# unirestore/UniRestore

Measured on AMD Instinct MI355X. Metric: restored 512x512 images/sec @ 20 denoise steps (whole job), higher is better.
Workload: dtype bf16; 1 GPU; PIR 512x512 batch=8/GPU, 20 DDIM steps, bf16, hipGraph replay (BASELINE.json configs[1]; configs[2] shape for N=8); global_batch=8, per_gpu_batch=8, image=512, denoise_steps=20, parallelism=image-parallel dp1, weights=seeded random init (no checkpoints reachable)

## Files before the change

### unirestore_amd/csrc/igemm.hip

```cpp
#include "igemm_impl.h"

namespace urk {
#define UR_DECLARE(name)                                                                                             \
  ConvLaunch name##_bf16(void* k, size_t ws_bytes);                                                                 \
  ConvLaunch name##_f16(void* k, size_t ws_bytes);                                                                  \
  static ConvLaunch name(ConvK& k, size_t ws_bytes) { return (k.f16 ? name##_f16 : name##_bf16)(&k, ws_bytes); }
UR_CONV_LAUNCHERS(UR_DECLARE)
#undef UR_DECLARE
}

namespace {

ConvLaunch dispatch_conv(ConvK& k, bool pair, size_t ws_bytes) {
  k.fold = 0;
  if (k.w4 && k.ups && k.KH == 3 && k.stride == 1 && k.pad_t == 1 && k.pad_l == 1 && k.kcm && k.staged_ok_ && !pair && k.nbatch == 1 &&
      k.C2 == 0 && k.Cin % 64 == 0 && k.W % 32 == 0 && k.H % 8 == 0 && k.OH == 2 * k.H && k.OW == 2 * k.W && !k.yt && !k.gn_ab && !k.row_stats &&
      !k.ln_stats) {
    k.fold = 1;
    const long long tm = 4ll * k.N * (k.H / 8) * (k.W / 32);
    auto fill = [](long long t) { return (double)t / (double)(((t + 255) / 256) * 256); };
    const bool ok128 = k.Cout % 128 == 0, ok160 = k.Cout % 160 == 0;
    if (ok160 && (!ok128 || fill(tm * (k.Cout / 160)) >= fill(tm * (k.Cout / 128)))) return urk::halo_8x32_160(k, ws_bytes);
    return urk::halo_8x32_128(k, ws_bytes);
  }
  if (k.KH == 3 && k.stride == 1 && k.pad_t == 1 && k.pad_l == 1 && k.kcm && k.staged_ok_ && !pair && k.nbatch == 1 &&
      k.OW % 32 == 0 && k.OH % 8 == 0 && k.OH == (k.ups ? 2 * k.H : k.H) && k.OW == (k.ups ? 2 * k.W : k.W) && !k.yt) {
    const bool ok128 = k.Cout % 128 == 0, ok160 = k.Cout % 160 == 0;
    const long long tm8 = (long long)k.N * (k.OH / 8) * (k.OW / 32);
    auto eff = [](long long t) { return t <= 128 ? (double)(t * (256 / t)) / 256.0 : (double)t / (double)(((t + 255) / 256) * 256); };
    const bool use160 = ok160 && (!ok128 || eff(tm8 * (k.Cout / 160)) >= eff(tm8 * (k.Cout / 128)));
    const long long tiles8 = tm8 * (use160 ? k.Cout / 160 : k.Cout / 128);
    if ((ok128 || ok160) && tiles8 >= 64) {
      if (use160) return urk::halo_8x32_160(k, ws_bytes);
      return urk::halo_8x32_128(k, ws_bytes);
    }
  }
  if (k.KH == 3 && k.stride == 1 && k.pad_t == 1 && k.pad_l == 1 && k.kcm && !pair && k.nbatch == 1 && !k.ups && k.C2 == 0 &&
      k.Cout <= 32 && k.OW % 32 == 0 && k.OH % 8 == 0 && k.OH == k.H && k.OW == k.W && !k.yt && !k.gn_part && !k.gn_ab && !k.row_stats && !k.ln_stats &&
      !k.bias_img && (long long)k.N * (k.OH / 8) * (k.OW / 32) >= 128)
    return urk::halo_thin_32(k, ws_bytes);
  const bool himg_ups = k.ups && k.OH == 16 && k.OW == 16 && k.H == 8 && k.W == 8;
  if (k.KH == 3 && k.stride == 1 && k.pad_t == 1 && k.pad_l == 1 && k.kcm && k.staged_ok_ && !pair && k.nbatch == 1 &&
      ((!k.ups && k.OH == k.H && k.OW == k.W) || himg_ups) && !k.yt && k.Cout % 128 == 0 && k.nk >= 36) {
    if (k.wf && k.OH == 8 && k.OW == 8 && k.N <= 16 && k.Cin % 256 == 0 && k.nk >= 72 && k.y && k.ws && !k.gn_ab && !k.row_stats && !k.ln_stats &&
        (long long)(k.nk / 36) * k.M * k.Cout * 4 <= (long long)ws_bytes)
      return urk::wstream_8x8(k, ws_bytes);
    if (k.OH == 16 && k.OW == 16) return urk::himg_16x16(k, ws_bytes);
    if (k.OH == 8 && k.OW == 8 && k.N % 4 == 0) {
      return urk::himg_8x8x4(k, ws_bytes);
    }
// ... 220 lines not shown
```

### unirestore_amd/csrc/igemm_impl.h

```cpp
#pragma once
#include <cstdio>
#include <cstdlib>
#include <map>
#include <string>

#include "common.h"

static __device__ uint4 g_zero_page[8];
typedef uint32_t ig_u32x4 __attribute__((ext_vector_type(4)));

struct ConvLaunch {
  int (*launch)(void* k, hipStream_t s);
  int prologue_ok;
  int id;
};

namespace {

struct ConvK {
  const uint16_t* x; const uint16_t* x2; const uint16_t* w; const float* bias; const uint16_t* res;
  void* y; uint16_t* yt; float* ws; float* gn_part; const float* gn_ab;
  float* row_stats; const float* ln_stats; const float* ln_colsum; float ln_eps; int ln_dim, ln_parts;
  int N, H, W, C1, ldx, C2, ldx2, Cin, Cout, ldw, ldy, ldr, KH, KW, stride, pad_t, pad_l, OH, OW, OHW;
  int ups, act, out_f32, n_split, t_rows, t_ld;
// ... 1862 lines not shown
    static ur::DeviceOnce attr_once;
    if (auto once_guard = attr_once.first()) {
      hipFuncSetAttribute(reinterpret_cast<const void*>(&igemm_halo_kernel<TH, BN, WM, WN, UR_TU_F16 != 0, false>), hipFuncAttributeMaxDynamicSharedMemorySize, lds);
      hipFuncSetAttribute(reinterpret_cast<const void*>(&igemm_halo_kernel<TH, BN, WM, WN, UR_TU_F16 != 0, GN_OK>), hipFuncAttributeMaxDynamicSharedMemorySize, lds);
      hipFuncSetAttribute(reinterpret_cast<const void*>(&igemm_halo_ws_kernel<TH, BN, WM, WN, UR_TU_F16 != 0, false>), hipFuncAttributeMaxDynamicSharedMemorySize, lds);
      hipFuncSetAttribute(reinterpret_cast<const void*>(&igemm_halo_ws_kernel<TH, BN, WM, WN, UR_TU_F16 != 0, GN_OK>), hipFuncAttributeMaxDynamicSharedMemorySize, lds);
      hipFuncSetAttribute(reinterpret_cast<const void*>(&igemm_halo_kernel<TH, BN, WM, WN, UR_TU_F16 != 0, false, 4>), hipFuncAttributeMaxDynamicSharedMemorySize, lds);
      hipFuncSetAttribute(reinterpret_cast<const void*>(&igemm_halo_ws_kernel<TH, BN, WM, WN, UR_TU_F16 != 0, false, 4>), hipFuncAttributeMaxDynamicSharedMemorySize, lds);
    }
    static const bool no_ws = getenv("UR_HALO_NOWS") != nullptr;
    if (k.fold) {
      const dim3 grid(k.tiles_m * k.tiles_n, 4);
      if (no_ws) UR_F16_SWITCH(k, hipLaunchKernelGGL((igemm_halo_kernel<TH, BN, WM, WN, F16, false, 4>), grid, dim3(NW * 64), lds, s, k));
      else UR_F16_SWITCH(k, hipLaunchKernelGGL((igemm_halo_ws_kernel<TH, BN, WM, WN, F16, false, 4>), grid, dim3((NW + 2) * 64), lds, s, k));
      return ur::check_launch("ur_conv2d_nhwc");
    }
    if (no_ws) {
      if (GN_OK && k.gn_ab) UR_F16_SWITCH(k, hipLaunchKernelGGL((igemm_halo_kernel<TH, BN, WM, WN, F16, GN_OK>), dim3(k.tiles_m * k.tiles_n, k.splitk), dim3(NW * 64), lds, s, k));
      else UR_F16_SWITCH(k, hipLaunchKernelGGL((igemm_halo_kernel<TH, BN, WM, WN, F16, false>), dim3(k.tiles_m * k.tiles_n, k.splitk), dim3(NW * 64), lds, s, k));
    } else {
      static const bool ld1 = getenv("UR_HALO_LD1") != nullptr;
      const dim3 blk((NW + (ld1 ? 1 : 2)) * 64);
      if (GN_OK && k.gn_ab) UR_F16_SWITCH(k, hipLaunchKernelGGL((igemm_halo_ws_kernel<TH, BN, WM, WN, F16, GN_OK>), dim3(k.tiles_m * k.tiles_n, k.splitk), blk, lds, s, k));
      else UR_F16_SWITCH(k, hipLaunchKernelGGL((igemm_halo_ws_kernel<TH, BN, WM, WN, F16, false>), dim3(k.tiles_m * k.tiles_n, k.splitk), blk, lds, s, k));
    }
    if (k.splitk > 1) {
      k.patch_tw = 0;
      launch_splitk_reduce(k, s);
    }
    return ur::check_launch("ur_conv2d_nhwc");
  }
};

template <int TH, int TW, int NIMG, int BN, int WM, int WN, bool F16, bool GNP>
__global__ __launch_bounds__(WM* WN * 64) void igemm_halo_img_kernel(const ConvK p) {
  constexpr int NW = WM * WN, BM = TH * TW * NIMG, PW = TW + 2, HP = (TH + 2) * PW, HPIX = HP * NIMG;
  constexpr int HSLOTS = (HPIX + 8 * NW - 1) / (8 * NW);
  constexpr int HPIECES = HSLOTS * NW, HBYTES = HPIECES * 1024;
  constexpr int WBYTES = BN * 128, WPIECES = BN / 8, WPW = (WPIECES + NW - 1) / NW;
  constexpr int WTM = BM / WM, WTN = BN / WN, FM = WTM / 32, FN = WTN / 32, NT = NW * 64;
  static_assert(BM == 256 && NW == 8 && WTM % 32 == 0 && WTN % 32 == 0 && HSLOTS <= 8, "tile shape");
  extern __shared__ __attribute__((aligned(16))) unsigned char smem[];
  unsigned char* const hbuf = smem;
  unsigned char* const wring = smem + 2 * HBYTES;
  unsigned char* const abuf = wring + 3 * WBYTES;
  constexpr bool GN_OK = NIMG == 1 && HSLOTS <= 7;
  constexpr bool gnp = GN_OK && GNP;

  const int tid = threadIdx.x, lane = tid & 63, wid = tid >> 6;
  const int wm = wid % WM, wn = wid / WM;
  int sz = blockIdx.y, tn, tmi;
  if (p.wmajor) {
    const int L = blockIdx.x, xcd = L & 7, j = L >> 3;
    const int g = (j / p.tiles_m) * 8 + xcd;
    if (g >= p.tiles_n * p.splitk) return;
    tn = g % p.tiles_n; sz = g / p.tiles_n; tmi = j % p.tiles_m;
  } else {
    int id = blockIdx.x;
    const int nt = p.tiles_m * p.tiles_n, q = nt >> 3, r = nt & 7, xcd = id & 7, idx = id >> 3;
    id = (xcd < r ? xcd * (q + 1) : r * (q + 1) + (xcd - r) * q) + idx;
    tn = id % p.tiles_n; tmi = id / p.tiles_n;
  }
  const int n0 = tn * BN, img0 = tmi * NIMG, m0 = tmi * BM;

  typedef __attribute__((address_space(1))) const void* gptr_t;
  typedef __attribute__((address_space(3))) void* lptr_t;
  const uint16_t* __restrict__ X1 = p.x;
  const uint16_t* __restrict__ X2 = p.x2;
  const uint16_t* __restrict__ Wt = p.w;
  const uint16_t* zero = reinterpret_cast<const uint16_t*>(g_zero_page);
  const int lr = lane >> 3, ps = lane & 7;

  int hpix[HSLOTS], hchk[HSLOTS];
#pragma unroll
  for (int t = 0; t < HSLOTS; ++t) {
    const int hr = (t * NW + wid) * 8 + lr;
    const int im = hr / HP, rin = hr - im * HP, hy = rin / PW, hx = rin - hy * PW;
    const int iy = hy - 1, ix = hx - 1;
    const bool v = hr < HPIX && img0 + im < p.N && (unsigned)iy < (unsigned)TH && (unsigned)ix < (unsigned)TW;
    const int sy = p.ups ? iy >> 1 : iy, sx = p.ups ? ix >> 1 : ix;
    hpix[t] = v ? ((img0 + im) * p.H + sy) * p.W + sx : -1;
    hchk[t] = ps ^ (((rin >> 1) - hy) & 7);
  }
  const int wchunk = ps ^ ((((wid & 1) << 2) + (lr >> 1)) & 7);
  int woff[WPW];
#pragma unroll
  for (int i = 0; i < WPW; ++i) {
    const int qq = (wid + NW * i < WPIECES) ? wid + NW * i : wid;
    const int row = n0 + qq * 8 + lr;
    woff[i] = row < p.Cout ? row * p.ldw : -1;
  }
  const int nchunk_all = p.nk / 9, cps = p.nk_per_split / 9;
  const int c_begin = sz * cps, c_end = min(nchunk_all, c_begin + cps);
  const int nchunk = c_end - c_begin, nk = nchunk * 9, kt0 = c_begin * 9;

  const int wid_s = __builtin_amdgcn_readfirstlane(wid);
  const ig_u32x4 rs_w = ig_make_rsrc(Wt, (unsigned long long)p.Cout * p.ldw * 2);
  const ig_u32x4 rs_x1 = ig_make_rsrc(X1, (unsigned long long)p.N * p.H * p.W * p.ldx * 2);
  const ig_u32x4 rs_x2 = ig_make_rsrc(X2 ? X2 : X1, (unsigned long long)p.N * p.H * p.W * (X2 ? p.ldx2 : p.ldx) * 2);
  const unsigned wring_lds = (unsigned)(uintptr_t)(lptr_t)wring, hbuf_lds = (unsigned)(uintptr_t)(lptr_t)hbuf;
  unsigned wvo[WPW];
#pragma unroll
  for (int i = 0; i < WPW; ++i) wvo[i] = woff[i] >= 0 ? (unsigned)woff[i] * 2u + wchunk * 16u : IG_OOB;
  auto issue_w = [&](int kt, int ring) {
#pragma unroll
    for (int i = 0; i < WPW; ++i) {
      const int qq = (wid_s + NW * i < WPIECES) ? wid_s + NW * i : wid_s;
      ig_lds_dma16(wring_lds + ring * WBYTES + qq * 1024, wvo[i], rs_w, (unsigned)(kt0 + kt) * 128u);
    }
  };
  auto issue_h = [&](int c, int t) {
    const int cb = (c_begin + c) * 64;
    const bool second = cb >= p.C1;
    const unsigned ld2 = (unsigned)(second ? p.ldx2 : p.ldx) * 2u;
    const unsigned vo = hpix[t] >= 0 ? (unsigned)hpix[t] * ld2 + hchk[t] * 16u : IG_OOB;
    const unsigned m0v = hbuf_lds + (c & 1) * HBYTES + (t * NW + wid_s) * 1024;
    if (second) ig_lds_dma16(m0v, vo, rs_x2, (unsigned)(cb - p.C1) * 2u);
    else ig_lds_dma16(m0v, vo, rs_x1, (unsigned)cb * 2u);
  };
  auto issue_ab = [&](int c) {
    const float* t = p.gn_ab + ((long long)img0 * 2 + (lane >> 4 & 1)) * p.Cin + (c_begin + c) * 64 + (lane & 15) * 4;
    const void* g = lane < 32 ? (const void*)t : (const void*)zero;
    __builtin_amdgcn_global_load_lds((gptr_t)g, (lptr_t)(abuf + (c & 1) * 1024), 16, 0, 0);
  };
  auto gn_slot = [&](int c, int t) {
    if (hpix[t] >= 0)
      gn_piece_inplace<F16>(hbuf + (c & 1) * HBYTES + (t * NW + wid) * 1024 + lane * 16, gn_load_ab(abuf + (c & 1) * 1024, hchk[t]), p.gn_silu != 0);
  };

  f32x16 acc[FN][FM];
// ... 4 lines not shown
#pragma unroll
      for (int e = 0; e < 16; ++e) acc[a][b][e] = 0.f;
  const int frow = lane & 31, fhalf = lane >> 5;
  int hrow0[FM], hin0[FM], hy0[FM];
#pragma unroll
  for (int b = 0; b < FM; ++b) {
    const int pix = wm * WTM + b * 32 + frow;
    const int im = pix / (TH * TW), r = pix - im * (TH * TW), y = r / TW, x = r - y * TW;
    hin0[b] = y * PW + x;
    hrow0[b] = im * HP + hin0[b];
    hy0[b] = y;
  }
  const unsigned hb_lds = (unsigned)(uintptr_t)(lptr_t)hbuf;
  const unsigned aw_lds = (unsigned)(uintptr_t)(lptr_t)wring + (wn * WTN + frow) * 128 + ((fhalf ^ ((frow >> 1) & 7)) << 4);
  static_assert(((WTN >> 1) & 7) == 0, "the wave's weight rows must keep the swizzle phase of fragment row 0");

  if (gnp) issue_ab(0);
#pragma unroll
  for (int t = 0; t < HSLOTS; ++t) issue_h(0, t);
  issue_w(0, 0);
  if (nk > 1) {
    issue_w(1, 1);
    asm volatile("s_waitcnt vmcnt(%0)" ::"n"(WPW) : "memory");
  } else {
    asm volatile("s_waitcnt vmcnt(0)" ::: "memory");
  }
  if (gnp) {
#pragma unroll
    for (int t = 0; t < HSLOTS; ++t) gn_slot(0, t);
    asm volatile("s_waitcnt lgkmcnt(0)" ::: "memory");
  }
  __builtin_amdgcn_s_barrier();

  for (int c = 0; c < nchunk; ++c) {
    const unsigned char* hb = hbuf + (c & 1) * HBYTES;
    const bool next_chunk = c + 1 < nchunk;
#pragma unroll
    for (int tap = 0; tap < 9; ++tap) {
      const int kt = c * 9 + tap;
      const bool more_w = kt + 2 < nk;
      const bool more_h = tap < HSLOTS && next_chunk;
      if (more_w) issue_w(kt + 2, (tap + 2) % 3);
      if (tap < HSLOTS) { if (next_chunk) issue_h(c + 1, tap < HSLOTS ? tap : 0); }
      const bool ab_now = gnp && tap == 0 && next_chunk;
      if (ab_now) issue_ab(c + 1);
      if (gnp && tap >= 2 && tap - 2 < HSLOTS && next_chunk) gn_slot(c + 1, (tap >= 2 && tap - 2 < HSLOTS) ? tap - 2 : 0);
      if constexpr (ktile_asm_ok<FM, FN>()) {
        const int dy = tap / 3, dx = tap % 3;
        unsigned ab[FM];
#pragma unroll
        for (int b = 0; b < FM; ++b) {
          const int hsw = (((hin0[b] + dy * PW + dx) >> 1) - (hy0[b] + dy)) & 7;
          ab[b] = hb_lds + (c & 1) * HBYTES + (hrow0[b] + dy * PW + dx) * 128 + ((fhalf ^ hsw) << 4);
        }
        ktile_mma<FM, FN, F16>(acc, ab, aw_lds + (tap % 3) * WBYTES);
      } else {
        const int dy = tap / 3, dx = tap % 3;
        const unsigned char* wsm = wring + (tap % 3) * WBYTES;
        int hro[FM], hsw[FM];
#pragma unroll
        for (int b = 0; b < FM; ++b) {
          hro[b] = (hrow0[b] + dy * PW + dx) * 128;
          hsw[b] = (((hin0[b] + dy * PW + dx) >> 1) - (hy0[b] + dy)) & 7;
        }
#pragma unroll
        for (int ks = 0; ks < 4; ++ks) {
          const int slot = ks * 2 + fhalf;
          typename Frag<F16>::type bfr[FM], afr[FN];
#pragma unroll
          for (int b = 0; b < FM; ++b) bfr[b] = *reinterpret_cast<const typename Frag<F16>::type*>(hb + hro[b] + ((slot ^ hsw[b]) << 4));
#pragma unroll
          for (int a = 0; a < FN; ++a) {
            const int row = wn * WTN + a * 32 + frow;
            afr[a] = *reinterpret_cast<const typename Frag<F16>::type*>(wsm + row * 128 + ((slot ^ ((row >> 1) & 7)) << 4));
          }
#pragma unroll
          for (int a = 0; a < FN; ++a)
#pragma unroll
            for (int b = 0; b < FM; ++b)
              acc[a][b] = mfma16t(afr[a], bfr[b], acc[a][b]);
        }
      }
      if (ab_now) {
        if (more_w) asm volatile("s_waitcnt vmcnt(%0)" ::"n"(WPW + 2) : "memory");
        else asm volatile("s_waitcnt vmcnt(2)" ::: "memory");
      } else if (more_w && more_h) asm volatile("s_waitcnt vmcnt(%0)" ::"n"(WPW + 1) : "memory");
      else if (more_w) asm volatile("s_waitcnt vmcnt(%0)" ::"n"(WPW) : "memory");
      else if (more_h) asm volatile("s_waitcnt vmcnt(1)" ::: "memory");
      else asm volatile("s_waitcnt vmcnt(0)" ::: "memory");
      asm volatile("s_waitcnt lgkmcnt(0)" ::: "memory");
      __builtin_amdgcn_s_barrier();
    }
  }
  asm volatile("s_nop 15\n\ts_nop 7" ::: "memory");
  igemm_epilogue<FM, FN, WTM, WTN, BM, BN, NT, F16, false>(p, acc, m0, n0, wm, wn, lane, 0, sz, smem);
}

template <int TH, int TW, int NIMG, int BN, int WM, int WN, bool F16>
__global__ __launch_bounds__((WM * WN + 2) * 64) void igemm_halo_img_ws_kernel(const ConvK p) {
  constexpr int NW = WM * WN, BM = TH * TW * NIMG, PW = TW + 2, HP = (TH + 2) * PW, HPIX = HP * NIMG;
  constexpr int HSLOTS = (HPIX + 8 * NW - 1) / (8 * NW);
  constexpr int HPIECES = HSLOTS * NW, HBYTES = HPIECES * 1024;
  constexpr int WBYTES = BN * 128, WPIECES = BN / 8;
  constexpr int WTM = BM / WM, WTN = BN / WN, FM = WTM / 32, FN = WTN / 32, NT = NW * 64;
  static_assert(BM == 256 && NW == 8 && WTM % 32 == 0 && WTN % 32 == 0 && HSLOTS <= 8 && ktile_asm_ok<FM, FN>() && WPIECES % NW == 0, "tile shape");
  extern __shared__ __attribute__((aligned(16))) unsigned char smem[];
  unsigned char* const hbuf = smem;
  unsigned char* const wring = smem + 2 * HBYTES;
  typedef __attribute__((address_space(3))) void* lptr_t;

  const int tid = threadIdx.x, lane = tid & 63, wid = tid >> 6;
  const int wid_s = __builtin_amdgcn_readfirstlane(wid);
  int sz = blockIdx.y, tn, tmi;
  if (p.wmajor) {
    const int L = blockIdx.x, xcd = L & 7, j = L >> 3;
    const int g = (j / p.tiles_m) * 8 + xcd;
    if (g >= p.tiles_n * p.splitk) return;
    tn = g % p.tiles_n; sz = g / p.tiles_n; tmi = j % p.tiles_m;
  } else {
    int id = blockIdx.x;
    const int nt = p.tiles_m * p.tiles_n, q = nt >> 3, r = nt & 7, xcd = id & 7, idx = id >> 3;
    id = (xcd < r ? xcd * (q + 1) : r * (q + 1) + (xcd - r) * q) + idx;
    tn = id % p.tiles_n; tmi = id / p.tiles_n;
  }
  const int n0 = tn * BN, img0 = tmi * NIMG, m0 = tmi * BM;
  const int lr = lane >> 3, ps = lane & 7;
  const int nchunk_all = p.nk / 9, cps = p.nk_per_split / 9;
  const int c_begin = sz * cps, c_end = min(nchunk_all, c_begin + cps);
  const int nchunk = c_end - c_begin, nk = nchunk * 9, kt0 = c_begin * 9;
  const ig_u32x4 rs_w = ig_make_rsrc(p.w, (unsigned long long)p.Cout * p.ldw * 2);
  const ig_u32x4 rs_x1 = ig_make_rsrc(p.x, (unsigned long long)p.N * p.H * p.W * p.ldx * 2);
  const ig_u32x4 rs_x2 = ig_make_rsrc(p.x2 ? p.x2 : p.x, (unsigned long long)p.N * p.H * p.W * (p.x2 ? p.ldx2 : p.ldx) * 2);
  const unsigned wring_lds = (unsigned)(uintptr_t)(lptr_t)wring, hbuf_lds = (unsigned)(uintptr_t)(lptr_t)hbuf;

  auto piece_of = [&](int q, int& pix, int& chk) {
    const int hr = q * 8 + lr;
    const int im = hr / HP, rin = hr - im * HP, hy = rin / PW, hx = rin - hy * PW;
    const int iy = hy - 1, ix = hx - 1;
    const bool v = hr < HPIX && img0 + im < p.N && (unsigned)iy < (unsigned)TH && (unsigned)ix < (unsigned)TW;
    const int sy = p.ups ? iy >> 1 : iy, sx = p.ups ? ix >> 1 : ix;
    pix = v ? ((img0 + im) * p.H + sy) * p.W + sx : -1;
    chk = ps ^ (((rin >> 1) - hy) & 7);
  };
  auto dma_piece = [&](int c, int q, int pix, int chk) {
    const int cb = (c_begin + c) * 64;
    const bool second = cb >= p.C1;
    const unsigned ld2 = (unsigned)(second ? p.ldx2 : p.ldx) * 2u;
    const unsigned vo = pix >= 0 ? (unsigned)pix * ld2 + chk * 16u : IG_OOB;
    const unsigned m0v = hbuf_lds + (c & 1) * HBYTES + q * 1024;
    if (second) ig_lds_dma16(m0v, vo, rs_x2, (unsigned)(cb - p.C1) * 2u);
    else ig_lds_dma16(m0v, vo, rs_x1, (unsigned)cb * 2u);
  };
  auto wvo_of = [&](int q) -> unsigned {
    const int row = n0 + q * 8 + lr;
    const int wchunk = ps ^ ((((q & 1) << 2) + (lr >> 1)) & 7);
    return row < p.Cout ? (unsigned)row * (unsigned)p.ldw * 2u + wchunk * 16u : IG_OOB;
  };

  if (wid_s == NW) {
    unsigned wvo[WPIECES];
#pragma unroll
    for (int q = 0; q < WPIECES; ++q) wvo[q] = wvo_of(q);
    auto dma_w = [&](int kt, int ring) {
      const unsigned so = (unsigned)(kt0 + kt) * 128u;
#pragma unroll
      for (int q = 0; q < WPIECES; ++q) ig_lds_dma16(wring_lds + ring * WBYTES + q * 1024, wvo[q], rs_w, so);
    };
    if (nk > 1) dma_w(1, 1);
    asm volatile("s_waitcnt vmcnt(0)" ::: "memory");
    __builtin_amdgcn_s_barrier();
    for (int kt = 0; kt < nk; ++kt) {
      if (kt + 2 < nk) {
        dma_w(kt + 2, (kt + 2) % 3);
        asm volatile("s_waitcnt vmcnt(%0)" ::"n"(WPIECES) : "memory");
      } else {
        asm volatile("s_waitcnt vmcnt(0)" ::: "memory");
      }
      __builtin_amdgcn_s_barrier();
    }
    return;
  }
  if (wid_s == NW + 1) {
    int hpx[HPIECES];
#pragma unroll
    for (int q = 0; q < HPIECES; ++q) { int pix, chk; piece_of(q, pix, chk); hpx[q] = pix >= 0 ? pix * 8 + chk : -1; }
    __builtin_amdgcn_s_barrier();
    constexpr int PPT = (HPIECES + 7) / 8;
    for (int c = 0; c < nchunk; ++c) {
      const bool next_chunk = c + 1 < nchunk;
#pragma unroll
      for (int tap = 0; tap < 9; ++tap) {
        if (next_chunk && tap < 8) {
#pragma unroll
          for (int j = 0; j < PPT; ++j) {
            const int q = tap * PPT + j;
            if (q < HPIECES) dma_piece(c + 1, q, hpx[q < HPIECES ? q : 0] >= 0 ? hpx[q < HPIECES ? q : 0] >> 3 : -1, hpx[q < HPIECES ? q : 0] & 7);
          }
        }
        if (tap == 8 || !next_chunk) asm volatile("s_waitcnt vmcnt(0)" ::: "memory");
        else asm volatile("s_waitcnt vmcnt(%0)" ::"n"(PPT) : "memory");
        __builtin_amdgcn_s_barrier();
      }
    }
    return;
  }

  const int wm = wid % WM, wn = wid / WM;
  {
#pragma unroll
    for (int t = 0; t < HSLOTS; ++t) { int pix, chk; piece_of(t * NW + wid_s, pix, chk); dma_piece(0, t * NW + wid_s, pix, chk); }
#pragma unroll
    for (int i = 0; i < WPIECES / NW; ++i) ig_lds_dma16(wring_lds + (wid_s + NW * i) * 1024, wvo_of(wid_s + NW * i), rs_w, (unsigned)kt0 * 128u);
  }
  f32x16 acc[FN][FM];
#pragma unroll
  for (int a = 0; a < FN; ++a)
#pragma unroll
    for (int b = 0; b < FM; ++b)
#pragma unroll
      for (int e = 0; e < 16; ++e) acc[a][b][e] = 0.f;
  const int frow = lane & 31, fhalf = lane >> 5;
  int hrow0[FM], hin0[FM], hy0[FM];
#pragma unroll
  for (int b = 0; b < FM; ++b) {
    const int pix = wm * WTM + b * 32 + frow;
    const int im = pix / (TH * TW), r = pix - im * (TH * TW), y = r / TW, x = r - y * TW;
    hin0[b] = y * PW + x;
    hrow0[b] = im * HP + hin0[b];
    hy0[b] = y;
  }
  const unsigned aw_lds = wring_lds + (wn * WTN + frow) * 128 + ((fhalf ^ ((frow >> 1) & 7)) << 4);
  static_assert(((WTN >> 1) & 7) == 0, "the wave's weight rows must keep the swizzle phase of fragment row 0");
  asm volatile("s_waitcnt vmcnt(0)" ::: "memory");
  __builtin_amdgcn_s_barrier();
  for (int c = 0; c < nchunk; ++c) {
#pragma unroll
    for (int tap = 0; tap < 9; ++tap) {
      const int dy = tap / 3, dx = tap % 3;
      unsigned ab[FM];
#pragma unroll
      for (int b = 0; b < FM; ++b) {
        const int hsw = (((hin0[b] + dy * PW + dx) >> 1) - (hy0[b] + dy)) & 7;
        ab[b] = hbuf_lds + (c & 1) * HBYTES + (hrow0[b] + dy * PW + dx) * 128 + ((fhalf ^ hsw) << 4);
      }
      ktile_mma<FM, FN, F16>(acc, ab, aw_lds + (tap % 3) * WBYTES);
      asm volatile("s_waitcnt lgkmcnt(0)" ::: "memory");
      __builtin_amdgcn_s_barrier();
    }
  }
  asm volatile("s_nop 15\n\ts_nop 7" ::: "memory");
  igemm_epilogue<FM, FN, WTM, WTN, BM, BN, NT, F16, false>(p, acc, m0, n0, wm, wn, lane, 0, sz, smem);
}

template <int TH, int TW, int NIMG, int BN, int WM, int WN>
struct HaloImg {
  static constexpr int NW = WM * WN, BM = TH * TW * NIMG, HPIX = (TH + 2) * (TW + 2) * NIMG, HSLOTS = (HPIX + 8 * NW - 1) / (8 * NW);
  static constexpr int HBYTES = HSLOTS * NW * 1024;
  static constexpr bool GN_OK = NIMG == 1 && HSLOTS <= 7;
  static constexpr int lds_loop = 2 * HBYTES + 3 * BN * 128 + (GN_OK ? 2048 : 0), lds_epi = epi_lds_bytes<BM, BN, NW * 64>();
  static constexpr int lds = lds_loop > lds_epi ? lds_loop : lds_epi;
  static_assert(lds <= 160 * 1024, "LDS budget");
  static int plan(ConvK& k, size_t ws_bytes) {
    k.tiles_m = (k.N + NIMG - 1) / NIMG;
    k.tiles_n = (k.Cout + BN - 1) / BN;
    const int nchunk = k.nk / 9;
    const long long tiles = (long long)k.tiles_m * k.tiles_n;
    plan_splitk(k, ws_bytes, tiles < 200 && k.ws && k.y ? std::min<long long>(std::max<long long>(256 / tiles, 1), std::max(1, nchunk / 2)) : 1, 9);
    set_gn_plan(k, (k.OHW % BM) == 0, k.OHW / BM);
    return GN_OK;
  }
  static int launch(ConvK& k, hipStream_t s) {
    static ur::DeviceOnce attr_once;
    if (auto once_guard = attr_once.first()) {
      hipFuncSetAttribute(reinterpret_cast<const void*>(&igemm_halo_img_kernel<TH, TW, NIMG, BN, WM, WN, UR_TU_F16 != 0, false>), hipFuncAttributeMaxDynamicSharedMemorySize, lds);
      hipFuncSetAttribute(reinterpret_cast<const void*>(&igemm_halo_img_kernel<TH, TW, NIMG, BN, WM, WN, UR_TU_F16 != 0, GN_OK>), hipFuncAttributeMaxDynamicSharedMemorySize, lds);
    }
    static const bool no_wmajor = getenv("UR_HIMG_NOWMAJOR") != nullptr;
    const int slices = k.tiles_n * k.splitk, per_xcd = ((slices + 7) / 8) * k.tiles_m;
    k.wmajor = !no_wmajor && (long long)k.Cout * k.Ktot > (long long)k.N * k.H * k.W * k.Cin && per_xcd <= 32 && slices >= 8;
    const dim3 grid = k.wmajor ? dim3(8 * per_xcd, 1) : dim3(k.tiles_m * k.tiles_n, k.splitk);
    static const bool himg_ws = getenv("UR_HIMG_NOWS") == nullptr;
    if (himg_ws && !k.gn_ab) {
      static ur::DeviceOnce ws_once;
      if (auto g2 = ws_once.first())
        hipFuncSetAttribute(reinterpret_cast<const void*>(&igemm_halo_img_ws_kernel<TH, TW, NIMG, BN, WM, WN, UR_TU_F16 != 0>), hipFuncAttributeMaxDynamicSharedMemorySize, lds);
      UR_F16_SWITCH(k, hipLaunchKernelGGL((igemm_halo_img_ws_kernel<TH, TW, NIMG, BN, WM, WN, F16>), grid, dim3((NW + 2) * 64), lds, s, k));
    } else if (GN_OK && k.gn_ab) UR_F16_SWITCH(k, hipLaunchKernelGGL((igemm_halo_img_kernel<TH, TW, NIMG, BN, WM, WN, F16, GN_OK>), grid, dim3(NW * 64), lds, s, k));
    else UR_F16_SWITCH(k, hipLaunchKernelGGL((igemm_halo_img_kernel<TH, TW, NIMG, BN, WM, WN, F16, false>), grid, dim3(NW * 64), lds, s, k));
    if (k.splitk > 1) launch_splitk_reduce(k, s);
    return ur::check_launch("ur_conv2d_nhwc");
  }
};

}
```

### unirestore_amd/ops.py

```python
from dataclasses import dataclass
from typing import Optional

import torch

from . import capi
from .capi import (UR_ACT_GATE, UR_ACT_GEGLU, UR_ACT_GELU, UR_ACT_NONE, UR_ACT_RELU, UR_ACT_SILU, UR_ACT_TANH, UR_DT_BF16,
                   UR_DT_F16, ConvDesc, ConvPlan, check, lib)

BF16 = torch.bfloat16
F16 = torch.float16
_ws = {}

_DTYPES = {"bf16": BF16, "bfloat16": BF16, BF16: BF16, "fp16": F16, "float16": F16, "f16": F16, "16": F16, F16: F16}
_act = BF16


def set_dtype(dt) -> torch.dtype:
    global _act
    if dt not in _DTYPES:
        raise ValueError(f"unsupported compute dtype {dt!r}: choose 'bf16' or 'fp16'")
    _act = _DTYPES[dt]
    return _act


def act_dtype() -> torch.dtype:
    return _act


def _dt(t: Optional[torch.Tensor] = None) -> int:
    d = _act if t is None else t.dtype
    if d == BF16:
        return UR_DT_BF16
# ... 58 lines not shown
        if self.w_frag is None:
            nt, nc = self.cout // 128, self.cin // 64
            w = self.w.view(nt, 4, 32, nc, 9, 4, 2, 8)
            self.w_frag = w.permute(0, 3, 4, 5, 1, 6, 2, 7).contiguous()
        return self.w_frag

    w_up4: Optional[torch.Tensor] = None

    def up4(self, weight: torch.Tensor) -> torch.Tensor:
        if self.w_up4 is None:
            w = weight.detach().to(self.w.device, torch.float32).permute(0, 2, 3, 1)
            if w.shape[0] != self.cout or w.shape[3] != self.cin:
                w = torch.nn.functional.pad(w, (0, self.cin - w.shape[3], 0, 0, 0, 0, 0, self.cout - w.shape[0]))
            self.w_up4 = up4_pack(up4_fold(w), self.w.dtype)
        return self.w_up4


def up4_fold(w: torch.Tensor) -> torch.Tensor:
    sel = w.new_tensor([[[1, 0, 0], [0, 1, 1]], [[1, 1, 0], [0, 0, 1]]])
    return torch.einsum("pay,qbx,oyxc->pqoabc", sel, sel, w)


def up4_pack(w4: torch.Tensor, dtype) -> torch.Tensor:
    _, _, cout, _, _, cin = w4.shape
    assert cin % 64 == 0
    return w4.to(dtype).reshape(4, cout, 4, cin // 64, 64).permute(0, 1, 3, 2, 4).reshape(4, cout, 4 * cin).contiguous()


def up4_unpack(packed: torch.Tensor, cin: int) -> torch.Tensor:
    cout = packed.shape[1]
    return packed.reshape(2, 2, cout, cin // 64, 2, 2, 64).permute(0, 1, 2, 4, 5, 3, 6).reshape(2, 2, cout, 2, 2, cin)


def wants_up4(pc: "PackedConv", n, h, w_, c1, c2, stride, upsample, groups, pad=(1, 1)) -> bool:
    return (pc.k == 3 and pc.kcm and groups == 1 and stride == 1 and bool(upsample) and tuple(pad) == (1, 1) and not pc.pair
            and c2 == 0 and c1 % 64 == 0 and w_ % 32 == 0 and h % 8 == 0)


def wants_frag(pc: "PackedConv", n, h, w_, c1, c2, stride, upsample, groups) -> bool:
    return (pc.k == 3 and pc.kcm and groups == 1 and stride == 1 and not upsample and h == 8 and w_ == 8 and n <= 16 and not pc.pair
            and pc.cout % 128 == 0 and (c1 + c2) % 256 == 0 and (c1 + c2) >= 512 and (c2 == 0 or c1 % 64 == 0))


def pack_conv(weight: torch.Tensor, bias: Optional[torch.Tensor], dev, *, pair=False, groups=1, cin_pad=None, c1=None, group_halo=False) -> PackedConv:
    w = weight.detach().to(dev, torch.float32)
    if w.dim() == 2:
        w = w[:, :, None, None]
    cout, cin_g, kh, kw = w.shape
    assert kh == kw and kh in (1, 3)
    cin_p = cin_pad or round_up(cin_g, 8)
    cout_p = round_up(cout, 8)
    if groups > 1:
        assert cin_g % 8 == 0 and (cout // groups) % 4 == 0
    if cin_p == cin_g and cout_p == cout:
        wp = w.permute(0, 2, 3, 1).contiguous()
    else:
        wp = torch.zeros(cout_p, kh, kw, cin_p, dtype=torch.float32, device=dev)
        wp[:cout, :, :, :cin_g] = w.permute(0, 2, 3, 1)
    b = None
    if bias is not None:
        b = torch.zeros(cout_p, dtype=torch.float32, device=dev)
        b[:cout] = bias.detach().to(dev, torch.float32)
    cout_out = cout_p
    if pair:
        half = cout // 2
        if cout % 2 or half % 32:
            raise NotImplementedError(f"UR_E_UNSUPPORTED: pair activations (GEGLU / SimpleGate) need (Cout/2) % 32 == 0, got {half}")
        idx = torch.arange(cout, device=dev).view(2, half // 32, 32).permute(1, 0, 2).reshape(-1)
        wp = wp[idx]
# ... 1024 lines not shown
```

Before: 30.43 images/s.

## Extend folded 4-tap upsample conv to 16x16 inputs via whole-image halo kernel

Adds a 4-tap phase-decomposed (nearest-upsample folded) variant of the whole-image halo implicit-GEMM kernels. For 16x16 inputs with Cin>=256 it is selected when enough workgroups exist. Each of the four output phases runs a 2x2 conv on the low-resolution input instead of a 3x3 conv on the upsampled image, which cuts MACs by about 9/4 and shrinks halo loads. The trade-offs are extra weight packing, new vmcnt wait cases and a rotating weight-ring index, plus a heuristic threshold that decides when the fold is worth it.

```diff
diff --git a/unirestore_amd/csrc/igemm.hip b/unirestore_amd/csrc/igemm.hip
--- a/unirestore_amd/csrc/igemm.hip
+++ b/unirestore_amd/csrc/igemm.hip
@@ -13,9 +13,16 @@
 
 ConvLaunch dispatch_conv(ConvK& k, bool pair, size_t ws_bytes) {
   k.fold = 0;
-  if (k.w4 && k.ups && k.KH == 3 && k.stride == 1 && k.pad_t == 1 && k.pad_l == 1 && k.kcm && k.staged_ok_ && !pair && k.nbatch == 1 &&
-      k.C2 == 0 && k.Cin % 64 == 0 && k.W % 32 == 0 && k.H % 8 == 0 && k.OH == 2 * k.H && k.OW == 2 * k.W && !k.yt && !k.gn_ab && !k.row_stats &&
-      !k.ln_stats) {
+  const bool fold_ok = k.w4 && k.ups && k.KH == 3 && k.stride == 1 && k.pad_t == 1 && k.pad_l == 1 && k.kcm && k.staged_ok_ && !pair && k.nbatch == 1 &&
+                       k.C2 == 0 && k.Cin % 64 == 0 && k.OH == 2 * k.H && k.OW == 2 * k.W && !k.yt && !k.gn_ab && !k.row_stats && !k.ln_stats;
+  if (fold_ok && k.H == 16 && k.W == 16 && k.Cin >= 256 && himg_up4_bn(k)) {
+    static const int min_wgs = getenv("UR_HIMG_FOLD_MIN") ? atoi(getenv("UR_HIMG_FOLD_MIN")) : 80;
+    if (4ll * k.N * (k.Cout / himg_up4_bn(k)) >= min_wgs || k.Cin <= 320) {
+      k.fold = 1;
+      return urk::himg_16x16(k, ws_bytes);
+    }
+  }
+  if (fold_ok && k.W % 32 == 0 && k.H % 8 == 0) {
     k.fold = 1;
     const long long tm = 4ll * k.N * (k.H / 8) * (k.W / 32);
     auto fill = [](long long t) { return (double)t / (double)(((t + 255) / 256) * 256); };
diff --git a/unirestore_amd/csrc/igemm_impl.h b/unirestore_amd/csrc/igemm_impl.h
--- a/unirestore_amd/csrc/igemm_impl.h
+++ b/unirestore_amd/csrc/igemm_impl.h
@@ -1918,8 +1918,10 @@
   }
 };
 
-template <int TH, int TW, int NIMG, int BN, int WM, int WN, bool F16, bool GNP>
+template <int TH, int TW, int NIMG, int BN, int WM, int WN, bool F16, bool GNP, int NTAP = 9>
 __global__ __launch_bounds__(WM* WN * 64) void igemm_halo_img_kernel(const ConvK p) {
+  constexpr bool UP4 = NTAP == 4;
+  static_assert((NTAP == 9 || NTAP == 4) && !(UP4 && (GNP || NIMG != 1)), "tap count");
   constexpr int NW = WM * WN, BM = TH * TW * NIMG, PW = TW + 2, HP = (TH + 2) * PW, HPIX = HP * NIMG;
   constexpr int HSLOTS = (HPIX + 8 * NW - 1) / (8 * NW);
   constexpr int HPIECES = HSLOTS * NW, HBYTES = HPIECES * 1024;
@@ -1932,6 +1934,8 @@
   unsigned char* const abuf = wring + 3 * WBYTES;
   constexpr bool GN_OK = NIMG == 1 && HSLOTS <= 7;
   constexpr bool gnp = GN_OK && GNP;
+  constexpr int HPT = UP4 ? (HSLOTS + NTAP - 2) / (NTAP - 1) : 1;
+  static_assert(HPT <= 2, "vmcnt cases of the tap wait");
 
   const int tid = threadIdx.x, lane = tid & 63, wid = tid >> 6;
   const int wm = wid % WM, wn = wid / WM;
@@ -1939,7 +1943,7 @@
   if (p.wmajor) {
     const int L = blockIdx.x, xcd = L & 7, j = L >> 3;
     const int g = (j / p.tiles_m) * 8 + xcd;
-    if (g >= p.tiles_n * p.splitk) return;
+    if (g >= p.tiles_n * (UP4 ? 4 : p.splitk)) return;
     tn = g % p.tiles_n; sz = g / p.tiles_n; tmi = j % p.tiles_m;
   } else {
     int id = blockIdx.x;
@@ -1947,13 +1951,16 @@
     id = (xcd < r ? xcd * (q + 1) : r * (q + 1) + (xcd - r) * q) + idx;
     tn = id % p.tiles_n; tmi = id / p.tiles_n;
   }
-  const int n0 = tn * BN, img0 = tmi * NIMG, m0 = tmi * BM;
+  const int phase = UP4 ? sz : 0, py = phase >> 1, px = phase & 1;
+  if constexpr (UP4) sz = 0;
+  const int n0 = tn * BN, img0 = tmi * NIMG, m0 = UP4 ? up4_m0(p, img0, 0, 0, TH, TW, py) : tmi * BM;
+  const int ldw = UP4 ? 4 * p.Cin : p.ldw;
 
   typedef __attribute__((address_space(1))) const void* gptr_t;
   typedef __attribute__((address_space(3))) void* lptr_t;
   const uint16_t* __restrict__ X1 = p.x;
   const uint16_t* __restrict__ X2 = p.x2;
-  const uint16_t* __restrict__ Wt = p.w;
+  const uint16_t* __restrict__ Wt = UP4 ? p.w4 + (long long)phase * p.Cout * ldw : p.w;
   const uint16_t* zero = reinterpret_cast<const uint16_t*>(g_zero_page);
   const int lr = lane >> 3, ps = lane & 7;
 
@@ -1964,7 +1971,7 @@
     const int im = hr / HP, rin = hr - im * HP, hy = rin / PW, hx = rin - hy * PW;
     const int iy = hy - 1, ix = hx - 1;
     const bool v = hr < HPIX && img0 + im < p.N && (unsigned)iy < (unsigned)TH && (unsigned)ix < (unsigned)TW;
-    const int sy = p.ups ? iy >> 1 : iy, sx = p.ups ? ix >> 1 : ix;
+    const int sy = !UP4 && p.ups ? iy >> 1 : iy, sx = !UP4 && p.ups ? ix >> 1 : ix;
     hpix[t] = v ? ((img0 + im) * p.H + sy) * p.W + sx : -1;
     hchk[t] = ps ^ (((rin >> 1) - hy) & 7);
   }
@@ -1974,14 +1981,14 @@
   for (int i = 0; i < WPW; ++i) {
     const int qq = (wid + NW * i < WPIECES) ? wid + NW * i : wid;
     const int row = n0 + qq * 8 + lr;
-    woff[i] = row < p.Cout ? row * p.ldw : -1;
-  }
-  const int nchunk_all = p.nk / 9, cps = p.nk_per_split / 9;
+    woff[i] = row < p.Cout ? row * ldw : -1;
+  }
+  const int nchunk_all = p.nk / NTAP, cps = p.nk_per_split / NTAP;
   const int c_begin = sz * cps, c_end = min(nchunk_all, c_begin + cps);
-  const int nchunk = c_end - c_begin, nk = nchunk * 9, kt0 = c_begin * 9;
+  const int nchunk = c_end - c_begin, nk = nchunk * NTAP, kt0 = c_begin * NTAP;
 
   const int wid_s = __builtin_amdgcn_readfirstlane(wid);
-  const ig_u32x4 rs_w = ig_make_rsrc(Wt, (unsigned long long)p.Cout * p.ldw * 2);
+  const ig_u32x4 rs_w = ig_make_rsrc(Wt, (unsigned long long)p.Cout * ldw * 2);
   const ig_u32x4 rs_x1 = ig_make_rsrc(X1, (unsigned long long)p.N * p.H * p.W * p.ldx * 2);
   const ig_u32x4 rs_x2 = ig_make_rsrc(X2 ? X2 : X1, (unsigned long long)p.N * p.H * p.W * (X2 ? p.ldx2 : p.ldx) * 2);
   const unsigned wring_lds = (unsigned)(uintptr_t)(lptr_t)wring, hbuf_lds = (unsigned)(uintptr_t)(lptr_t)hbuf;
@@ -2052,31 +2059,42 @@
   }
   __builtin_amdgcn_s_barrier();
 
+  int r0 = 0;
   for (int c = 0; c < nchunk; ++c) {
     const unsigned char* hb = hbuf + (c & 1) * HBYTES;
     const bool next_chunk = c + 1 < nchunk;
 #pragma unroll
-    for (int tap = 0; tap < 9; ++tap) {
-      const int kt = c * 9 + tap;
+    for (int tap = 0; tap < NTAP; ++tap) {
+      const int kt = c * NTAP + tap;
+      const int r1 = r0 == 2 ? 0 : r0 + 1, r2 = r1 == 2 ? 0 : r1 + 1;
       const bool more_w = kt + 2 < nk;
-      const bool more_h = tap < HSLOTS && next_chunk;
-      if (more_w) issue_w(kt + 2, (tap + 2) % 3);
-      if (tap < HSLOTS) { if (next_chunk) issue_h(c + 1, tap < HSLOTS ? tap : 0); }
+      const bool more_h = (UP4 ? tap * HPT < HSLOTS && tap < NTAP - 1 : tap < HSLOTS) && next_chunk;
+      const int nh = !UP4 ? 1 : (tap + 1) * HPT <= HSLOTS ? HPT : HSLOTS - tap * HPT;
+      if (more_w) issue_w(kt + 2, UP4 ? r2 : (tap + 2) % 3);
+      if constexpr (UP4) {
+        if (more_h) {
+#pragma unroll
+          for (int j = 0; j < HPT; ++j)
+            if (tap * HPT + j < HSLOTS) issue_h(c + 1, tap * HPT + j < HSLOTS ? tap * HPT + j : 0);
+        }
+      } else {
+        if (tap < HSLOTS) { if (next_chunk) issue_h(c + 1, tap < HSLOTS ? tap : 0); }
+      }
       const bool ab_now = gnp && tap == 0 && next_chunk;
       if (ab_now) issue_ab(c + 1);
       if (gnp && tap >= 2 && tap - 2 < HSLOTS && next_chunk) gn_slot(c + 1, (tap >= 2 && tap - 2 < HSLOTS) ? tap - 2 : 0);
       if constexpr (ktile_asm_ok<FM, FN>()) {
-        const int dy = tap / 3, dx = tap % 3;
+        const int dy = UP4 ? py + tap / 2 : tap / 3, dx = UP4 ? px + tap % 2 : tap % 3;
         unsigned ab[FM];
 #pragma unroll
         for (int b = 0; b < FM; ++b) {
           const int hsw = (((hin0[b] + dy * PW + dx) >> 1) - (hy0[b] + dy)) & 7;
           ab[b] = hb_lds + (c & 1) * HBYTES + (hrow0[b] + dy * PW + dx) * 128 + ((fhalf ^ hsw) << 4);
         }
-        ktile_mma<FM, FN, F16>(acc, ab, aw_lds + (tap % 3) * WBYTES);
+        ktile_mma<FM, FN, F16>(acc, ab, aw_lds + (UP4 ? r0 : tap % 3) * WBYTES);
       } else {
-        const int dy = tap / 3, dx = tap % 3;
-        const unsigned char* wsm = wring + (tap % 3) * WBYTES;
+        const int dy = UP4 ? py + tap / 2 : tap / 3, dx = UP4 ? px + tap % 2 : tap % 3;
+        const unsigned char* wsm = wring + (UP4 ? r0 : tap % 3) * WBYTES;
         int hro[FM], hsw[FM];
 #pragma unroll
         for (int b = 0; b < FM; ++b) {
@@ -2104,26 +2122,36 @@
       if (ab_now) {
         if (more_w) asm volatile("s_waitcnt vmcnt(%0)" ::"n"(WPW + 2) : "memory");
         else asm volatile("s_waitcnt vmcnt(2)" ::: "memory");
-      } else if (more_w && more_h) asm volatile("s_waitcnt vmcnt(%0)" ::"n"(WPW + 1) : "memory");
+      } else if (more_w && more_h && nh == 2) asm volatile("s_waitcnt vmcnt(%0)" ::"n"(WPW + 2) : "memory");
+      else if (more_w && more_h) asm volatile("s_waitcnt vmcnt(%0)" ::"n"(WPW + 1) : "memory");
       else if (more_w) asm volatile("s_waitcnt vmcnt(%0)" ::"n"(WPW) : "memory");
+      else if (more_h && nh == 2) asm volatile("s_waitcnt vmcnt(2)" ::: "memory");
       else if (more_h) asm volatile("s_waitcnt vmcnt(1)" ::: "memory");
       else asm volatile("s_waitcnt vmcnt(0)" ::: "memory");
       asm volatile("s_waitcnt lgkmcnt(0)" ::: "memory");
       __builtin_amdgcn_s_barrier();
+      if constexpr (UP4) r0 = r1;
     }
   }
   asm volatile("s_nop 15\n\ts_nop 7" ::: "memory");
-  igemm_epilogue<FM, FN, WTM, WTN, BM, BN, NT, F16, false>(p, acc, m0, n0, wm, wn, lane, 0, sz, smem);
-}
-
-template <int TH, int TW, int NIMG, int BN, int WM, int WN, bool F16>
+  if constexpr (UP4) {
+    const ConvK q = up4_out_view(p, py, px, 1);
+    igemm_epilogue<FM, FN, WTM, WTN, BM, BN, NT, F16, false>(q, acc, m0, n0, wm, wn, lane, 0, 0, smem);
+  } else {
+    igemm_epilogue<FM, FN, WTM, WTN, BM, BN, NT, F16, false>(p, acc, m0, n0, wm, wn, lane, 0, sz, smem);
+  }
+}
+
+template <int TH, int TW, int NIMG, int BN, int WM, int WN, bool F16, int NTAP = 9>
 __global__ __launch_bounds__((WM * WN + 2) * 64) void igemm_halo_img_ws_kernel(const ConvK p) {
+  constexpr bool UP4 = NTAP == 4;
+  static_assert((NTAP == 9 || NTAP == 4) && !(UP4 && NIMG != 1), "tap count");
   constexpr int NW = WM * WN, BM = TH * TW * NIMG, PW = TW + 2, HP = (TH + 2) * PW, HPIX = HP * NIMG;
   constexpr int HSLOTS = (HPIX + 8 * NW - 1) / (8 * NW);
   constexpr int HPIECES = HSLOTS * NW, HBYTES = HPIECES * 1024;
   constexpr int WBYTES = BN * 128, WPIECES = BN / 8;
   constexpr int WTM = BM / WM, WTN = BN / WN, FM = WTM / 32, FN = WTN / 32, NT = NW * 64;
-  static_assert(BM == 256 && NW == 8 && WTM % 32 == 0 && WTN % 32 == 0 && HSLOTS <= 8 && ktile_asm_ok<FM, FN>() && WPIECES % NW == 0, "tile shape");
+  static_assert(BM == 256 && NW == 8 && WTM % 32 == 0 && WTN % 32 == 0 && HSLOTS <= 8 && ktile_asm_ok<FM, FN>(), "tile shape");
   extern __shared__ __attribute__((aligned(16))) unsigned char smem[];
   unsigned char* const hbuf = smem;
   unsigned char* const wring = smem + 2 * HBYTES;
@@ -2135,7 +2163,7 @@
   if (p.wmajor) {
     const int L = blockIdx.x, xcd = L & 7, j = L >> 3;
     const int g = (j / p.tiles_m) * 8 + xcd;
-    if (g >= p.tiles_n * p.splitk) return;
+    if (g >= p.tiles_n * (UP4 ? 4 : p.splitk)) return;
     tn = g % p.tiles_n; sz = g / p.tiles_n; tmi = j % p.tiles_m;
   } else {
     int id = blockIdx.x;
@@ -2143,12 +2171,16 @@
     id = (xcd < r ? xcd * (q + 1) : r * (q + 1) + (xcd - r) * q) + idx;
     tn = id % p.tiles_n; tmi = id / p.tiles_n;
   }
-  const int n0 = tn * BN, img0 = tmi * NIMG, m0 = tmi * BM;
+  const int phase = UP4 ? sz : 0, py = phase >> 1, px = phase & 1;
+  if constexpr (UP4) sz = 0;
+  const int n0 = tn * BN, img0 = tmi * NIMG, m0 = UP4 ? up4_m0(p, img0, 0, 0, TH, TW, py) : tmi * BM;
+  const int ldw = UP4 ? 4 * p.Cin : p.ldw;
+  const uint16_t* const Wt = UP4 ? p.w4 + (long long)phase * p.Cout * ldw : p.w;
   const int lr = lane >> 3, ps = lane & 7;
-  const int nchunk_all = p.nk / 9, cps = p.nk_per_split / 9;
+  const int nchunk_all = p.nk / NTAP, cps = p.nk_per_split / NTAP;
   const int c_begin = sz * cps, c_end = min(nchunk_all, c_begin + cps);
-  const int nchunk = c_end - c_begin, nk = nchunk * 9, kt0 = c_begin * 9;
-  const ig_u32x4 rs_w = ig_make_rsrc(p.w, (unsigned long long)p.Cout * p.ldw * 2);
+  const int nchunk = c_end - c_begin, nk = nchunk * NTAP, kt0 = c_begin * NTAP;
+  const ig_u32x4 rs_w = ig_make_rsrc(Wt, (unsigned long long)p.Cout * ldw * 2);
   const ig_u32x4 rs_x1 = ig_make_rsrc(p.x, (unsigned long long)p.N * p.H * p.W * p.ldx * 2);
   const ig_u32x4 rs_x2 = ig_make_rsrc(p.x2 ? p.x2 : p.x, (unsigned long long)p.N * p.H * p.W * (p.x2 ? p.ldx2 : p.ldx) * 2);
   const unsigned wring_lds = (unsigned)(uintptr_t)(lptr_t)wring, hbuf_lds = (unsigned)(uintptr_t)(lptr_t)hbuf;
@@ -2158,7 +2190,7 @@
     const int im = hr / HP, rin = hr - im * HP, hy = rin / PW, hx = rin - hy * PW;
     const int iy = hy - 1, ix = hx - 1;
     const bool v = hr < HPIX && img0 + im < p.N && (unsigned)iy < (unsigned)TH && (unsigned)ix < (unsigned)TW;
-    const int sy = p.ups ? iy >> 1 : iy, sx = p.ups ? ix >> 1 : ix;
+    const int sy = !UP4 && p.ups ? iy >> 1 : iy, sx = !UP4 && p.ups ? ix >> 1 : ix;
     pix = v ? ((img0 + im) * p.H + sy) * p.W + sx : -1;
     chk = ps ^ (((rin >> 1) - hy) & 7);
   };
@@ -2174,7 +2206,7 @@
   auto wvo_of = [&](int q) -> unsigned {
     const int row = n0 + q * 8 + lr;
     const int wchunk = ps ^ ((((q & 1) << 2) + (lr >> 1)) & 7);
-    return row < p.Cout ? (unsigned)row * (unsigned)p.ldw * 2u + wchunk * 16u : IG_OOB;
+    return row < p.Cout ? (unsigned)row * (unsigned)ldw * 2u + wchunk * 16u : IG_OOB;
   };
 
   if (wid_s == NW) {
@@ -2205,19 +2237,19 @@
 #pragma unroll
     for (int q = 0; q < HPIECES; ++q) { int pix, chk; piece_of(q, pix, chk); hpx[q] = pix >= 0 ? pix * 8 + chk : -1; }
     __builtin_amdgcn_s_barrier();
-    constexpr int PPT = (HPIECES + 7) / 8;
+    constexpr int HN = UP4 ? (HPIX + 7) / 8 : HPIECES, PPT = (HN + NTAP - 2) / (NTAP - 1);
     for (int c = 0; c < nchunk; ++c) {
       const bool next_chunk = c + 1 < nchunk;
 #pragma unroll
-      for (int tap = 0; tap < 9; ++tap) {
-        if (next_chunk && tap < 8) {
+      for (int tap = 0; tap < NTAP; ++tap) {
+        if (next_chunk && tap < NTAP - 1) {
 #pragma unroll
           for (int j = 0; j < PPT; ++j) {
             const int q = tap * PPT + j;
-            if (q < HPIECES) dma_piece(c + 1, q, hpx[q < HPIECES ? q : 0] >= 0 ? hpx[q < HPIECES ? q : 0] >> 3 : -1, hpx[q < HPIECES ? q : 0] & 7);
+            if (q < HN) dma_piece(c + 1, q, hpx[q < HPIECES ? q : 0] >= 0 ? hpx[q < HPIECES ? q : 0] >> 3 : -1, hpx[q < HPIECES ? q : 0] & 7);
           }
         }
-        if (tap == 8 || !next_chunk) asm volatile("s_waitcnt vmcnt(0)" ::: "memory");
+        if (tap == NTAP - 1 || !next_chunk) asm volatile("s_waitcnt vmcnt(0)" ::: "memory");
         else asm volatile("s_waitcnt vmcnt(%0)" ::"n"(PPT) : "memory");
         __builtin_amdgcn_s_barrier();
       }
@@ -2230,7 +2262,8 @@
 #pragma unroll
     for (int t = 0; t < HSLOTS; ++t) { int pix, chk; piece_of(t * NW + wid_s, pix, chk); dma_piece(0, t * NW + wid_s, pix, chk); }
 #pragma unroll
-    for (int i = 0; i < WPIECES / NW; ++i) ig_lds_dma16(wring_lds + (wid_s + NW * i) * 1024, wvo_of(wid_s + NW * i), rs_w, (unsigned)kt0 * 128u);
+    for (int i = 0; i < (WPIECES + NW - 1) / NW; ++i)
+      if (WPIECES % NW == 0 || wid_s + NW * i < WPIECES) ig_lds_dma16(wring_lds + (wid_s + NW * i) * 1024, wvo_of(wid_s + NW * i), rs_w, (unsigned)kt0 * 128u);
   }
   f32x16 acc[FN][FM];
 #pragma unroll
@@ -2253,24 +2286,73 @@
   static_assert(((WTN >> 1) & 7) == 0, "the wave's weight rows must keep the swizzle phase of fragment row 0");
   asm volatile("s_waitcnt vmcnt(0)" ::: "memory");
   __builtin_amdgcn_s_barrier();
+  int r0 = 0;
   for (int c = 0; c < nchunk; ++c) {
 #pragma unroll
-    for (int tap = 0; tap < 9; ++tap) {
-      const int dy = tap / 3, dx = tap % 3;
+    for (int tap = 0; tap < NTAP; ++tap) {
+      const int dy = UP4 ? py + tap / 2 : tap / 3, dx = UP4 ? px + tap % 2 : tap % 3;
       unsigned ab[FM];
 #pragma unroll
       for (int b = 0; b < FM; ++b) {
         const int hsw = (((hin0[b] + dy * PW + dx) >> 1) - (hy0[b] + dy)) & 7;
         ab[b] = hbuf_lds + (c & 1) * HBYTES + (hrow0[b] + dy * PW + dx) * 128 + ((fhalf ^ hsw) << 4);
       }
-      ktile_mma<FM, FN, F16>(acc, ab, aw_lds + (tap % 3) * WBYTES);
+      ktile_mma<FM, FN, F16>(acc, ab, aw_lds + (UP4 ? r0 : tap % 3) * WBYTES);
       asm volatile("s_waitcnt lgkmcnt(0)" ::: "memory");
       __builtin_amdgcn_s_barrier();
+      if constexpr (UP4) r0 = r0 == 2 ? 0 : r0 + 1;
     }
   }
   asm volatile("s_nop 15\n\ts_nop 7" ::: "memory");
-  igemm_epilogue<FM, FN, WTM, WTN, BM, BN, NT, F16, false>(p, acc, m0, n0, wm, wn, lane, 0, sz, smem);
-}
+  if constexpr (UP4) {
+    const ConvK q = up4_out_view(p, py, px, 1);
+    igemm_epilogue<FM, FN, WTM, WTN, BM, BN, NT, F16, false>(q, acc, m0, n0, wm, wn, lane, 0, 0, smem);
+  } else {
+    igemm_epilogue<FM, FN, WTM, WTN, BM, BN, NT, F16, false>(p, acc, m0, n0, wm, wn, lane, 0, sz, smem);
+  }
+}
+
+static inline int himg_up4_bn(const ConvK& k) {
+  static const int force_bn = getenv("UR_HIMG_FOLD_BN") ? atoi(getenv("UR_HIMG_FOLD_BN")) : 0;
+  const bool ok128 = k.Cout % 128 == 0, ok160 = k.Cout % 160 == 0;
+  if (!ok128 && !ok160) return 0;
+  if (ok128 && ok160 && (force_bn == 128 || force_bn == 160)) return force_bn;
+  auto fill = [](long long t) { return (double)t / (double)(((t + 255) / 256) * 256); };
+  const long long tm = 4ll * k.N;
+  return ok160 && (!ok128 || fill(tm * (k.Cout / 160)) >= fill(tm * (k.Cout / 128))) ? 160 : 128;
+}
+template <int TH, int TW, int BN, int WM, int WN>
+struct HaloImgUp4 {
+  static constexpr int NW = WM * WN, BM = TH * TW, HPIX = (TH + 2) * (TW + 2), HSLOTS = (HPIX + 8 * NW - 1) / (8 * NW);
+  static constexpr int HBYTES = HSLOTS * NW * 1024;
+  static constexpr int lds_loop = 2 * HBYTES + 3 * BN * 128, lds_epi = epi_lds_bytes<BM, BN, NW * 64>();
+  static constexpr int lds = lds_loop > lds_epi ? lds_loop : lds_epi;
+  static_assert(lds <= 160 * 1024, "LDS budget");
+  static void plan(ConvK& k) {
+    k.tiles_m = k.N;
+    k.tiles_n = k.Cout / BN;
+    k.nk = (k.Cin / 64) * 4;
+    k.splitk = 1;
+    k.nk_per_split = k.nk;
+    set_gn_plan(k, true, 4);
+  }
+  static int launch(ConvK& k, hipStream_t s) {
+    k.patch_tw = TW;
+    static ur::DeviceOnce attr_once;
+    if (auto once_guard = attr_once.first()) {
+      hipFuncSetAttribute(reinterpret_cast<const void*>(&igemm_halo_img_kernel<TH, TW, 1, BN, WM, WN, UR_TU_F16 != 0, false, 4>), hipFuncAttributeMaxDynamicSharedMemorySize, lds);
+      hipFuncSetAttribute(reinterpret_cast<const void*>(&igemm_halo_img_ws_kernel<TH, TW, 1, BN, WM, WN, UR_TU_F16 != 0, 4>), hipFuncAttributeMaxDynamicSharedMemorySize, lds);
+    }
+    static const bool no_wmajor = getenv("UR_HIMG_NOWMAJOR") != nullptr;
+    const int slices = k.tiles_n * 4, per_xcd = ((slices + 7) / 8) * k.tiles_m;
+    k.wmajor = !no_wmajor && 16ll * k.Cout > (long long)k.N * k.H * k.W && per_xcd <= 32 && slices >= 8;
+    const dim3 grid = k.wmajor ? dim3(8 * per_xcd, 1) : dim3(k.tiles_m * k.tiles_n, 4);
+    static const bool himg_ws = getenv("UR_HIMG_NOWS") == nullptr;
+    if (himg_ws) UR_F16_SWITCH(k, hipLaunchKernelGGL((igemm_halo_img_ws_kernel<TH, TW, 1, BN, WM, WN, F16, 4>), grid, dim3((NW + 2) * 64), lds, s, k));
+    else UR_F16_SWITCH(k, hipLaunchKernelGGL((igemm_halo_img_kernel<TH, TW, 1, BN, WM, WN, F16, false, 4>), grid, dim3(NW * 64), lds, s, k));
+    return ur::check_launch("ur_conv2d_nhwc");
+  }
+};
 
 template <int TH, int TW, int NIMG, int BN, int WM, int WN>
 struct HaloImg {
@@ -2281,6 +2363,13 @@
   static constexpr int lds = lds_loop > lds_epi ? lds_loop : lds_epi;
   static_assert(lds <= 160 * 1024, "LDS budget");
   static int plan(ConvK& k, size_t ws_bytes) {
+    if constexpr (NIMG == 1) {
+      if (k.fold) {
+        if (himg_up4_bn(k) == 160) HaloImgUp4<TH, TW, 160, 8, 1>::plan(k);
+        else HaloImgUp4<TH, TW, BN, WM, WN>::plan(k);
+        return 0;
+      }
+    }
     k.tiles_m = (k.N + NIMG - 1) / NIMG;
     k.tiles_n = (k.Cout + BN - 1) / BN;
     const int nchunk = k.nk / 9;
@@ -2290,6 +2379,9 @@
     return GN_OK;
   }
   static int launch(ConvK& k, hipStream_t s) {
+    if constexpr (NIMG == 1) {
+      if (k.fold) return k.Cout / k.tiles_n == 160 ? HaloImgUp4<TH, TW, 160, 8, 1>::launch(k, s) : HaloImgUp4<TH, TW, BN, WM, WN>::launch(k, s);
+    }
     static ur::DeviceOnce attr_once;
     if (auto once_guard = attr_once.first()) {
       hipFuncSetAttribute(reinterpret_cast<const void*>(&igemm_halo_img_kernel<TH, TW, NIMG, BN, WM, WN, UR_TU_F16 != 0, false>), hipFuncAttributeMaxDynamicSharedMemorySize, lds);
diff --git a/unirestore_amd/ops.py b/unirestore_amd/ops.py
--- a/unirestore_amd/ops.py
+++ b/unirestore_amd/ops.py
@@ -1,3 +1,4 @@
+import os
 from dataclasses import dataclass
 from typing import Optional
 
@@ -122,9 +123,20 @@
     return packed.reshape(2, 2, cout, cin // 64, 2, 2, 64).permute(0, 1, 2, 4, 5, 3, 6).reshape(2, 2, cout, 2, 2, cin)
 
 
+UP4_IMG_MIN_WGS = int(os.environ.get("UR_HIMG_FOLD_MIN", 80))
+
+
 def wants_up4(pc: "PackedConv", n, h, w_, c1, c2, stride, upsample, groups, pad=(1, 1)) -> bool:
-    return (pc.k == 3 and pc.kcm and groups == 1 and stride == 1 and bool(upsample) and tuple(pad) == (1, 1) and not pc.pair
-            and c2 == 0 and c1 % 64 == 0 and w_ % 32 == 0 and h % 8 == 0)
+    if not (pc.k == 3 and pc.kcm and groups == 1 and stride == 1 and bool(upsample) and tuple(pad) == (1, 1) and not pc.pair
+            and c2 == 0 and c1 % 64 == 0):
+        return False
+    if h == 16 and w_ == 16:
+        if c1 < 256 or (pc.cout % 128 and pc.cout % 160):
+            return False
+        fill = lambda t: t / (-(-t // 256) * 256)
+        bn = 160 if pc.cout % 160 == 0 and (pc.cout % 128 or fill(4 * n * (pc.cout // 160)) >= fill(4 * n * (pc.cout // 128))) else 128
+        return 4 * n * (pc.cout // bn) >= UP4_IMG_MIN_WGS or c1 <= 320
+    return w_ % 32 == 0 and h % 8 == 0
 
 
 def wants_frag(pc: "PackedConv", n, h, w_, c1, c2, stride, upsample, groups) -> bool:
```

After: 30.63 images/s (median of 6 runs). No clear change (+0.7%).
